# sachaMorin/dino

Hardware: AMD Instinct MI355X
Metric: frames/sec (480x480, ViT-S/8) DINOSeg inference (higher is better)
Workload: dtype fp16 (linears, Q.K^T; P.V bf16; fp32 accumulate)

## Files before the change

dino_amd/capi.py:

```python
from __future__ import annotations

import ctypes as C
import os
import re
from typing import Optional

import torch

_HERE = os.path.dirname(os.path.abspath(__file__))
LIB_PATH = os.path.join(_HERE, "lib", "libdinoseg_hip.so")
HEADER_PATH = os.path.join(os.path.dirname(_HERE), "include", "dinoseg.h")

BF16, BF16X3, FP16, FP16X3 = 0, 1, 2, 3
HEAD_LINEAR, HEAD_MLP = 0, 1
INPUT_U8_HWC, INPUT_F32_CHW = 0, 1
EPI_PLAIN, EPI_RESID, EPI_GELU, EPI_RELU = 0, 1, 2, 3
PROF_CLASSES = ("patch_embed", "layernorm", "qkv_gemm", "attention", "proj_gemm", "fc1_gemm", "fc2_gemm", "head", "attention_bwd")


class DinosegError(RuntimeError):
    pass


class Config(C.Structure):
# ... 54 lines not shown
                                              _i32, _i32, _i32, _f32, _i32, _i32, _vp]),
    "dinoseg_op_proj_pack_elems": (_i64, [_i32]),
    "dinoseg_op_pack_proj": (C.c_int, [_fp, _i32, _vp, _vp]),
    "dinoseg_op_proj_mlp_fused": (C.c_int, [_fp, _vp, _vp, _fp, _fp, _fp, _f32, _vp, _fp, _fp, _i32, _i32, _i32, _vp]),
    "dinoseg_op_pack_rs": (C.c_int, [_fp, _i32, _i32, _i32, _vp, _vp]),
    "dinoseg_op_gemm_rs": (C.c_int, [_vp, _i32, _vp, _fp, _i32, _i32, _i32, _i32, _fp, _vp, _i32, _vp, _vp, _vp, _i32, _i32, _i32, _f32, _vp]),
    "dinoseg_op_pack_rs_ln": (C.c_int, [_fp, _fp, _fp, _fp, _i32, _i32, _vp, _fp, _vp]),
    "dinoseg_op_ln_gemm_rs": (C.c_int, [_fp, _f32, _vp, _fp, _i32, _i32, _i32, _i32, _vp, _i32, _vp, _vp, _vp, _i32, _i32, _i32, _f32, _vp]),
    "dinoseg_op_mlp3_pack_elems": (_i64, [_i32, _i32]),
    "dinoseg_op_pack_mlp3": (C.c_int, [_fp, _fp, _fp, _fp, _fp, _fp, _fp, _fp, _fp, _fp, _i32, _i32, _i32, _vp, _vp]),
    "dinoseg_op_proj_mlp_fused3": (C.c_int, [_fp, _vp, _i64, _fp, _f32, _vp, _fp, _i32, _i32, _i32, _i32, _vp]),
    "dinoseg_op_mlp4_pack_elems": (_i64, [_i32, _i32]),
    "dinoseg_op_pack_mlp4": (C.c_int, [_fp, _fp, _fp, _fp, _fp, _fp, _fp, _fp, _fp, _fp, _i32, _i32, _i32, _vp, _vp]),
    "dinoseg_op_proj_mlp_fused4": (C.c_int, [_fp, _vp, _fp, _f32, _vp, _fp, _i32, _i32, _i32, _i32, _vp]),
    "dinoseg_op_block_tail_fused4": (C.c_int, [_fp, _vp, _fp, _f32, _vp, _fp, _vp, _vp, _vp, _i32, _i32, _i32, _i32, _f32, _i32, _i32, _i32, _vp]),
    "dinoseg_op_block_tail_fused3": (C.c_int, [_fp, _vp, _i64, _fp, _f32, _vp, _fp, _vp, _vp, _vp, _i64, _i32, _i32, _i32, _i32, _f32, _i32, _i32,
                                               _i32, _i32, _vp]),
    "dinoseg_op_attention": (C.c_int, [_vp, _vp, _vp, _i64, _vp, _i64, _fp, _i32, _i32, _i32, _i32, _i32, _vp]),
    "dinoseg_op_layernorm": (C.c_int, [_fp, _fp, _fp, _f32, _i32, _i32, _vp, _i64, _i32, _fp, _i32, _i32, _vp]),
    "dinoseg_op_pos_resample": (C.c_int, [_fp, _i32, _i32, _i32, _fp, _vp]),
    "dinoseg_op_patch_gather": (C.c_int, [_vp, _i32, _i32, _i32, _vp, _i64, _i32, _vp]),
    "dinoseg_op_head_final": (C.c_int, [_vp, _i64, _i32, _i32, _i32, _fp, _fp, _i32, _fp, _fp, _vp]),
    "dinoseg_op_head_wide": (C.c_int, [_vp, _i64, _i32, _i32, _i32, _vp, _i64, _fp, _i32, _fp, _fp, _vp]),
    "dinoseg_prepare_resolution_hw": (C.c_int, [_vp, _i32, _i32, _vp]),
    "dinoseg_forward_hw": (C.c_int, [_vp, _vp, _i32, _i32, _i32, _i32, _fp, _fp, _i32, _fp, _vp]),
    "dinoseg_last_selfattention_hw": (C.c_int, [_vp, _vp, _i32, _i32, _i32, _i32, _fp, _vp]),
    "dinoseg_forward_mask_hw": (C.c_int, [_vp, _vp, _i32, _i32, _i32, _fp, _i32, _fp, _fp, _vp]),
    "dinoseg_features_hw": (C.c_int, [_vp, _vp, _i32, _i32, _i32, _i32, _i32, _fp, _vp]),
    "dinoseg_train_forward_hw": (C.c_int, [_vp, _vp, _i32, _i32, _i32, _i32, _fp, _vp]),
    "dinoseg_train_step_hw": (C.c_int, [_vp, _vp, _i32, _i32, _i32, _i32, _fp, _fp, _fp, _vp]),
    "dinoseg_workspace_bytes_hw": (_i64, [_vp, _i32, _i32, _i32]),
    "dinoseg_op_pos_resample_hw": (C.c_int, [_fp, _i32, _i32, _i32, _i32, _fp, _vp]),
    "dinoseg_op_patch_gather_hw": (C.c_int, [_vp, _i32, _i32, _i32, _i32, _vp, _i64, _i32, _vp]),
}

_lib: Optional[C.CDLL] = None


def header_symbols() -> list:
    with open(HEADER_PATH) as f:
        text = re.sub(r"/\*.*?\*/", "", f.read(), flags=re.S)
    return sorted(set(re.findall(r"\b(dinoseg_[a-z0-9_]+)\s*\(", text)))


def lib() -> C.CDLL:
    global _lib
# ... 35 lines not shown
```

dino_amd/csrc/api.hip:

```cpp
#include <stdarg.h>
#include <stdio.h>
#include <string.h>

#include <map>
#include <string>
#include <vector>

#include "handle.h"

using namespace dseg;

static thread_local char g_err[1024] = "";

extern "C" void dinoseg_set_error(const char* fmt, ...) {
    va_list ap;
    va_start(ap, fmt);
    vsnprintf(g_err, sizeof(g_err), fmt, ap);
    va_end(ap);
}
extern "C" const char* dinoseg_last_error(void) { return g_err; }
extern "C" int dinoseg_version(void) { return 300; }

int device_cu_count() {
    static std::atomic<int> cache[64];
// ... 140 lines not shown
            return -1;
        }
        if (h->device != attr.device) {
            if (h->device >= 0) {
                DeviceGuard old(h);
                if (h->wbuf) (void)hipFree(h->wbuf);
                if (h->pos_cache) (void)hipFree(h->pos_cache);
                release_workspaces(h);
                (void)dinoseg_train_release(h);
                for (auto& e : h->stage_ev) (void)hipEventDestroy(e);
                h->stage_ev.clear();
                h->stage_done = 0;
                for (auto& r : h->prof_recs) {
                    (void)hipEventDestroy(r.a);
                    (void)hipEventDestroy(r.b);
                }
                h->prof_recs.clear();
                for (auto& e : h->prof_pool) (void)hipEventDestroy(e);
                h->prof_pool.clear();
                h->wbuf = nullptr; h->pos_cache = nullptr; h->pos_hp = h->pos_wp = -1;
                h->wbuf_bytes = h->pos_cap = 0;
                h->tws_B = h->tws_H = h->tws_W = h->tr_B = -1;
                h->packed.clear();
                h->packed_slab.clear();
                h->packed_mlp.clear();
                h->packed_proj.clear();
                h->packed_qkvf.clear();
                h->packed_mlp3.clear();
    h->packed_mlp4.clear();
    h->packed_rs_bias.clear();
                h->packed_mlp4.clear();
                h->packed_rs_bias.clear();
                h->packed_rs.clear();
                h->bound.clear();
                h->grads.clear();
            }
            h->device = attr.device;
        }
    }
    BoundTensor t;
    t.ptr = reinterpret_cast<const float*>(dev_ptr);
    t.shape.assign(shape, shape + ndim);
    h->bound[name] = t;
    h->weights_ready = false;
    h->pos_stale = true;
    return 0;
// ... 57 lines not shown
        if (ln_fed(sp)) total += align_up((size_t)gemm_ln_slab_elems(sp.N, sp.K, sp.planes) * sizeof(bf16_t), 256);
    }
    const int Dm = h->cfg.embed_dim, Fh = h->cfg.embed_dim * h->cfg.mlp_ratio;
    const bool mlp_fusable = mlp_fused_supported(Dm, Fh, h->planes);
    const bool mlp3_fusable = mlp_fused3_supported(Dm, Fh, h->planes);
    const bool mlp4_fusable = options().mlp_fused4 && mlp_fused4_supported(Dm, Fh, h->planes);
    auto rs_kind = [&](const LinSpec& sp) -> int {
        if (!options().gemm_rs || h->planes != 1 || Dm != 768 || sp.wname.rfind("dino.blocks.", 0) != 0) return -1;
        const int bit = sp.wname.find("mlp.fc1.weight") != std::string::npos ? 1 : sp.wname.find("attn.qkv.weight") != std::string::npos ? 2 : 4;
        if (!(options().gemm_rs & bit)) return -1;
        if (sp.K == 768 && (sp.wname.find("attn.qkv.weight") != std::string::npos || sp.wname.find("mlp.fc1.weight") != std::string::npos)) return 0;
        if (sp.N == 768 && sp.K % 192 == 0 && (sp.wname.find("attn.proj.weight") != std::string::npos || sp.wname.find("mlp.fc2.weight") != std::string::npos)) return 1;
        return -1;
    };
    auto rs_ln = [&](const LinSpec& sp) -> bool { return rs_kind(sp) == 0 && options().gemm_rs_ln; };
    for (const LinSpec& sp : specs)
        if (rs_kind(sp) >= 0) total += align_up((size_t)sp.N * sp.K * sizeof(bf16_t), 256) + (rs_ln(sp) ? align_up((size_t)sp.N * sizeof(float), 256) : 0);
    if (mlp3_fusable) total += (size_t)h->cfg.n_blocks * align_up((size_t)mlp_fused3_pack_elems(Dm, Fh) * sizeof(bf16_t), 256);
    if (mlp4_fusable) total += (size_t)h->cfg.n_blocks * align_up((size_t)mlp_fused4_pack_elems(Dm, Fh) * sizeof(bf16_t), 256);
    if (mlp_fusable)
        total += (size_t)h->cfg.n_blocks * (align_up((size_t)mlp_fused_pack_elems(Dm, Fh) * sizeof(bf16_t), 256) +
                                            align_up((size_t)mlp_fused_proj_pack_elems(Dm) * sizeof(bf16_t), 256) +
                                            align_up((size_t)mlp_fused_qkv_pack_elems(Dm) * sizeof(bf16_t), 256));
    if (total > h->wbuf_bytes) {
        ++h->generation;
        if (h->wbuf) DSEG_CHECK_HIP(hipFree(h->wbuf));
        h->wbuf = nullptr;
        DSEG_CHECK_HIP(hipMalloc(reinterpret_cast<void**>(&h->wbuf), total));
        h->wbuf_bytes = total;
    }
    size_t off = 0;
    std::vector<PackJob> jobs;
    for (const LinSpec& sp : specs) {
        PackedLinear pk;
        pk.w = reinterpret_cast<bf16_t*>(h->wbuf + off);
        pk.plane = (long)sp.n_pad * sp.k_pad;
        pk.n_pad = sp.n_pad;
        pk.k_pad = sp.k_pad;
        off += align_up((size_t)sp.planes * sp.n_pad * sp.k_pad * sizeof(bf16_t), 256);
        jobs.push_back({W(h, sp.wname), pk.w, pk.plane, sp.N, sp.K, sp.n_pad, sp.k_pad, sp.planes, 0, sp.fmt});
        if (sp.n_pad != sp.N) {
            pk.bias_pad = reinterpret_cast<float*>(h->wbuf + off);
            off += align_up((size_t)sp.n_pad * sizeof(float), 256);
            DSEG_CHECK_HIP(hipMemsetAsync(pk.bias_pad, 0, (size_t)sp.n_pad * sizeof(float), s));
            DSEG_CHECK_HIP(hipMemcpyAsync(pk.bias_pad, W(h, sp.bname), (size_t)sp.N * sizeof(float),
                                          hipMemcpyDeviceToDevice, s));
        }
        h->packed[sp.wname] = pk;
        if (ln_fed(sp)) {
            bf16_t* slab = reinterpret_cast<bf16_t*>(h->wbuf + off);
            off += align_up((size_t)gemm_ln_slab_elems(sp.N, sp.K, sp.planes) * sizeof(bf16_t), 256);
            DSEG_TRY(launch_pack_slabs(W(h, sp.wname), sp.N, sp.K, sp.planes, slab, s, sp.fmt));
            h->packed_slab[sp.wname] = slab;
        }
    }
    DSEG_TRY(launch_multi_pack(jobs.data(), (int)jobs.size(), s));
    h->packed_mlp.clear();
    h->packed_proj.clear();
    h->packed_qkvf.clear();
    h->packed_mlp3.clear();
    h->packed_rs.clear();
    for (const LinSpec& sp : specs)
        if (rs_kind(sp) >= 0) {
            bf16_t* dst = reinterpret_cast<bf16_t*>(h->wbuf + off);
            off += align_up((size_t)sp.N * sp.K * sizeof(bf16_t), 256);
            if (rs_ln(sp)) {
                float* fb = reinterpret_cast<float*>(h->wbuf + off);
                off += align_up((size_t)sp.N * sizeof(float), 256);
                const std::string blk = sp.wname.substr(0, sp.wname.find(sp.wname.find("attn.qkv") != std::string::npos ? "attn.qkv" : "mlp.fc1"));
                const std::string nrm = blk + (sp.wname.find("attn.qkv") != std::string::npos ? "norm1" : "norm2");
                DSEG_TRY(launch_pack_rs_ln(W(h, sp.wname), W(h, nrm + ".weight"), W(h, nrm + ".bias"), W(h, sp.bname), sp.N, sp.K, dst, fb, s, sp.fmt));
                h->packed_rs_bias[sp.wname] = fb;
            } else {
                DSEG_TRY(launch_pack_rs(W(h, sp.wname), sp.N, sp.K, rs_kind(sp), dst, s, sp.fmt));
            }
            h->packed_rs[sp.wname] = dst;
        }
    if (mlp3_fusable)
        for (int i = 0; i < h->cfg.n_blocks; ++i) {
// ... 445 lines not shown
            DSEG_PROF(DINOSEG_PROF_FC1, DSEG_TRY(gemm_any(g, b + "mlp.fc1.weight")));
        }
        }
        {
            const PackedLinear& pk = h->packed.at(b + "mlp.fc2.weight");
            GemmParams g = {};
            g.A = HB; g.a_plane = L.hb_plane; g.lda = F;
            g.W = pk.w; g.w_plane = pk.plane;
            g.M = L.M; g.N = D; g.K = F; g.planes = P; g.fmt = FM; g.epi = EPI_RESID; g.dispatch_rows = disp_M;
            g.bias = W(h, b + "mlp.fc2.bias");
            g.out_f32 = X; g.ldo_f32 = D;
            DSEG_PROF(DINOSEG_PROF_FC2, DSEG_TRY(gemm_any(g, b + "mlp.fc2.weight")));
        }
        }
        if (tap_block == i + 1 && tap_out) DSEG_CHECK_HIP(hipMemcpyAsync(tap_out, X, xbytes, hipMemcpyDeviceToDevice, s));
        if (mreq && mreq->feat_out && mreq->feat_blocks == i + 1 && i + 1 < c.n_blocks)
            return launch_layernorm(X, W(h, "dino.norm.weight"), W(h, "dino.norm.bias"), c.ln_eps, L.M, D, nullptr, 0, 1, mreq->feat_out, 0,
                                    L.ntok, s);
    }
    if (mreq && mreq->feat_out)
        return launch_layernorm(X, W(h, "dino.norm.weight"), W(h, "dino.norm.bias"), c.ln_eps, L.M, D, nullptr, 0, 1, mreq->feat_out, 0,
                                L.ntok, s);

    DSEG_PROF(DINOSEG_PROF_LN, DSEG_TRY(launch_layernorm(X, W(h, "dino.norm.weight"), W(h, "dino.norm.bias"), c.ln_eps, L.M, D, FEAT, L.feat_plane,
                              HP, nullptr, 1, L.ntok, s, SF)));

    if (c.head_kind == DINOSEG_HEAD_MLP) {
        {
            const PackedLinear& pk = h->packed.at("clf.layer_1.weight");
            GemmParams g = {};
            g.A = FEAT; g.a_plane = L.feat_plane; g.lda = D;
            g.W = pk.w; g.w_plane = pk.plane;
            g.M = L.Mp; g.N = 256; g.K = D; g.planes = HP; g.fmt = SF; g.epi = EPI_RELU;
            g.bias = pk.bias_pad;
            g.out_bf16 = H1; g.out_plane = L.h1_plane; g.ldo = 256;
            DSEG_PROF(DINOSEG_PROF_HEAD, DSEG_TRY(launch_gemm(g, s)));
        }
        {
            const PackedLinear& pk = h->packed.at("clf.layer_2.weight");
            GemmParams g = {};
            g.A = H1; g.a_plane = L.h1_plane; g.lda = 256;
            g.W = pk.w; g.w_plane = pk.plane;
            g.M = L.Mp; g.N = 128; g.K = 256; g.planes = HP; g.fmt = SF; g.epi = EPI_RELU;
            g.bias = pk.bias_pad;
            g.out_bf16 = H2; g.out_plane = L.h2_plane; g.ldo = 128;
            DSEG_PROF(DINOSEG_PROF_HEAD, DSEG_TRY(launch_gemm(g, s)));
// ... 577 lines not shown
extern "C" int dinoseg_op_patch_gather_hw(const void* x, int32_t x_kind, int32_t B, int32_t H, int32_t W, void* out, int64_t out_plane,
                                          int32_t planes, void* stream) {
    if (!frame_ok(H, W)) {
        dinoseg_set_error("Resolution should be a multiple of 8.");
        return -1;
    }
    float mean255[3], inv255[3];
    norm_consts(mean255, inv255);
    return launch_patch_gather(x, x_kind, B, H, W, mean255, inv255, reinterpret_cast<bf16_t*>(out), out_plane, planes,
                               reinterpret_cast<hipStream_t>(stream), planes == 2 ? options().op_fmt : FMT_BF16);
}

extern "C" int dinoseg_op_patch_gather(const void* x, int32_t x_kind, int32_t B, int32_t r, void* out, int64_t out_plane,
                                       int32_t planes, void* stream) {
    return dinoseg_op_patch_gather_hw(x, x_kind, B, r, r, out, out_plane, planes, stream);
}

extern "C" int dinoseg_op_head_final(const void* in, int64_t in_plane, int32_t ld, int32_t M, int32_t K, const float* Wc,
                                     const float* b, int32_t C, float* logp, int32_t* argmax, void* stream) {
    return launch_head_final(reinterpret_cast<const bf16_t*>(in), in_plane, ld, M, K, Wc, b, C, logp, argmax,
                             reinterpret_cast<hipStream_t>(stream), options().op_fmt);
}

extern "C" int dinoseg_op_head_wide(const void* in, int64_t in_plane, int32_t ld, int32_t M, int32_t K, const void* Wp, int64_t w_plane,
                                    const float* b, int32_t C, float* logp, int32_t* argmax, void* stream) {
    return launch_head_wide(reinterpret_cast<const bf16_t*>(in), in_plane, ld, M, K, reinterpret_cast<const bf16_t*>(Wp), w_plane, b, C,
                            logp, argmax, reinterpret_cast<hipStream_t>(stream), options().op_fmt);
}
```

dino_amd/csrc/common.h:

```cpp
#pragma once
#include <hip/hip_runtime.h>
#include <stdint.h>

namespace dseg {

typedef __attribute__((ext_vector_type(8))) __bf16 bf16x8;
typedef __attribute__((ext_vector_type(4))) __bf16 bf16x4;
typedef __attribute__((ext_vector_type(2))) __bf16 bf16x2;
typedef __attribute__((ext_vector_type(2))) float f32x2;
typedef __attribute__((ext_vector_type(4))) float f32x4;
typedef __attribute__((ext_vector_type(16))) float f32x16;

typedef uint16_t bf16_t;

constexpr int WAVE = 64;

__device__ __forceinline__ uint32_t pack_bf16x2(float a, float b) {
    f32x2 v = {a, b};
    return __builtin_bit_cast(uint32_t, __builtin_convertvector(v, bf16x2));
}
__device__ __forceinline__ float bf16_lo_to_f32(uint32_t packed) { return __builtin_bit_cast(float, packed << 16); }
__device__ __forceinline__ float bf16_hi_to_f32(uint32_t packed) { return __builtin_bit_cast(float, packed & 0xFFFF0000u); }
__device__ __forceinline__ float bf16_to_f32(bf16_t v) { return __builtin_bit_cast(float, (uint32_t)v << 16); }

// ... 68 lines not shown

__device__ __forceinline__ f32x16 mfma32(bf16x8 a, bf16x8 b, f32x16 c) {
    return __builtin_amdgcn_mfma_f32_32x32x16_bf16(a, b, c, 0, 0, 0);
}

template <int FMT>
__device__ __forceinline__ f32x16 mfma32f(bf16x8 a, bf16x8 b, f32x16 c) {
    if constexpr (FMT == FMT_FP16) return __builtin_amdgcn_mfma_f32_32x32x16_f16(__builtin_bit_cast(f16x8, a), __builtin_bit_cast(f16x8, b), c, 0, 0, 0);
    else return __builtin_amdgcn_mfma_f32_32x32x16_bf16(a, b, c, 0, 0, 0);
}

__device__ __forceinline__ bf16x8 lds_frag(const char* p) {
    return __builtin_bit_cast(bf16x8, *reinterpret_cast<const uint4*>(p));
}

__device__ __forceinline__ int acc_row(int r, int h) { return (r & 3) + 8 * (r >> 2) + 4 * h; }

__device__ __forceinline__ float wave_sum(float v) {
#pragma unroll
    for (int o = 32; o > 0; o >>= 1) v += __shfl_xor(v, o);
    return v;
}

__device__ __forceinline__ float gelu_erf(float x) {
    const float z = fabsf(x) * 0.70710678118654752440f;
    const float t = __builtin_amdgcn_rcpf(fmaf(0.3275911f, z, 1.0f));
    float pl = fmaf(1.061405429f, t, -1.453152027f);
    pl = fmaf(pl, t, 1.421413741f);
    pl = fmaf(pl, t, -0.284496736f);
    pl = fmaf(pl, t, 0.254829592f);
    const float pe = pl * t * __builtin_amdgcn_exp2f(-z * z * 1.44269504088896340736f);
    return 0.5f * x * (x >= 0.f ? 2.0f - pe : pe);
}

__device__ __forceinline__ float gelu_fast(float x) {
    const float xc = __builtin_amdgcn_fmed3f(x, -8.0f, 8.0f);
    const float u = xc * xc;
    float q = fmaf(1.01537542e-3f, u, -1.06782573e-1f);
    q = fmaf(q, u, -2.30111381f);
    const float e = __builtin_amdgcn_exp2f(q * xc);
    return x * __builtin_amdgcn_rcpf(1.0f + e);
}

__device__ __forceinline__ float gelu_erf_grad(float x) {
    const float z = fabsf(x) * 0.70710678118654752440f;
    const float t = __builtin_amdgcn_rcpf(fmaf(0.3275911f, z, 1.0f));
// ... 42 lines not shown
```

dino_amd/csrc/elementwise.hip:

```cpp
#include "common.h"
#include "kernels.h"

namespace dseg {

__global__ void pack_planes_kernel(const float* __restrict__ src, int rows, int cols, bf16_t* __restrict__ dst,
                                   long plane, int rows_pad, int cols_pad, int planes, int fmt) {
    const long total = (long)rows_pad * cols_pad;
    for (long i = (long)blockIdx.x * blockDim.x + threadIdx.x; i < total; i += (long)gridDim.x * blockDim.x) {
        const int r = (int)(i / cols_pad), c = (int)(i - (long)r * cols_pad);
        const float v = (r < rows && c < cols) ? src[(long)r * cols + c] : 0.f;
        bf16_t hi, lo;
        split1(v, fmt, hi, lo);
        dst[i] = hi;
        if (planes == 2) dst[plane + i] = lo;
    }
}

int launch_pack_planes(const float* src, int rows, int cols, bf16_t* dst, long plane, int rows_pad, int cols_pad,
                       int planes, hipStream_t s, int fmt) {
    const long total = (long)rows_pad * cols_pad;
    int grid = (int)((total + 255) / 256);
    if (grid > 2048) grid = 2048;
    hipLaunchKernelGGL(pack_planes_kernel, dim3(grid), dim3(256), 0, s, src, rows, cols, dst, plane, rows_pad, cols_pad, planes, fmt);
    DSEG_CHECK_HIP(hipGetLastError());
// ... 82 lines not shown
__global__ __launch_bounds__(256) void layernorm_kernel(const float* __restrict__ x, const float* __restrict__ gamma,
                                                        const float* __restrict__ beta, float eps, int M,
                                                        bf16_t* __restrict__ out, long out_plane, int planes,
                                                        float* __restrict__ out_f32, int drop_cls, int ntok, int fmt) {
    constexpr int D = 128 * NV;
    const int lane = threadIdx.x & 63;
    const int wid = blockIdx.x * 4 + (threadIdx.x >> 6);
    const int nw = gridDim.x * 4;
    f32x2 g[NV], bta[NV];
#pragma unroll
    for (int i = 0; i < NV; ++i) {
        g[i] = *reinterpret_cast<const f32x2*>(gamma + i * 128 + lane * 2);
        bta[i] = *reinterpret_cast<const f32x2*>(beta + i * 128 + lane * 2);
    }
    for (int m = wid; m < M; m += nw) {
        long orow = m;
        if (drop_cls) {
            const int b = m / ntok, t = m - b * ntok;
            if (t == 0) continue;
            orow = (long)b * (ntok - 1) + t - 1;
        }
        const float* xr = x + (long)m * D;
        f32x2 v[NV];
        float s = 0.f;
#pragma unroll
        for (int i = 0; i < NV; ++i) {
            v[i] = *reinterpret_cast<const f32x2*>(xr + i * 128 + lane * 2);
            s += v[i][0] + v[i][1];
        }
        const float mean = wave_sum(s) * (1.0f / D);
        float q = 0.f;
#pragma unroll
        for (int i = 0; i < NV; ++i) {
            v[i][0] -= mean;
            v[i][1] -= mean;
            q += v[i][0] * v[i][0] + v[i][1] * v[i][1];
        }
        const float rstd = 1.0f / sqrtf(wave_sum(q) * (1.0f / D) + eps);
#pragma unroll
        for (int i = 0; i < NV; ++i) {
            const float y0 = v[i][0] * rstd * g[i][0] + bta[i][0];
            const float y1 = v[i][1] * rstd * g[i][1] + bta[i][1];
            const long o = orow * D + i * 128 + lane * 2;
            if (out_f32) {
                f32x2 y = {y0, y1};
                *reinterpret_cast<f32x2*>(out_f32 + o) = y;
            }
            if (out) {
                uint32_t hi, lo;
                if (fmt == FMT_FP16) split2<FMT_FP16>(y0, y1, hi, lo);
                else split_bf16x2(y0, y1, hi, lo);
                *reinterpret_cast<uint32_t*>(out + o) = hi;
                if (planes == 2) *reinterpret_cast<uint32_t*>(out + out_plane + o) = lo;
            }
        }
    }
}

int launch_layernorm(const float* x, const float* gamma, const float* beta, float eps, int M, int D, bf16_t* out,
                     long out_plane, int planes, float* out_f32, int drop_cls, int ntok, hipStream_t s, int fmt) {
    if (M <= 0) return 0;
    if (D % 128 != 0 || D > 1024) {
        dinoseg_set_error("layernorm: D=%d must be a multiple of 128 and <= 1024", D);
        return -1;
    }
// ... 519 lines not shown
```

dino_amd/csrc/handle.h:

```cpp
#pragma once
#include <map>
#include <string>
#include <vector>

#include "../../include/dinoseg.h"
#include "common.h"
#include "kernels.h"

using namespace dseg;

#define DSEG_TRY(expr)            \
    do {                          \
        int _rc = (expr);         \
        if (_rc != 0) return _rc; \
    } while (0)

struct BoundTensor {
    const float* ptr = nullptr;
    std::vector<int64_t> shape;
};

struct PackedLinear {
    bf16_t* w = nullptr;
    long plane = 0;
    int n_pad = 0, k_pad = 0;
    float* bias_pad = nullptr;
};

struct dinoseg_handle {
    dinoseg_config cfg;
    int planes;
    int fmt = 0;
    int device = -1;
    std::map<std::string, BoundTensor> bound;
    std::map<std::string, std::vector<int64_t>> expected;
    char* wbuf = nullptr;
    size_t wbuf_bytes = 0;
    std::map<std::string, PackedLinear> packed;
    std::map<std::string, bf16_t*> packed_slab;
    std::map<std::string, bf16_t*> packed_mlp;
    std::map<std::string, bf16_t*> packed_proj;
    std::map<std::string, bf16_t*> packed_rs;
    std::map<std::string, float*> packed_rs_bias;
    std::map<std::string, bf16_t*> packed_mlp4;
    std::map<std::string, bf16_t*> packed_mlp3;
    std::map<std::string, bf16_t*> packed_qkvf;
    bool packed_mlp_stale = false;
    bool weights_ready = false;
    int fp16_patch_planes_snap = 1;
    int64_t generation = 0;
    float* pos_cache = nullptr;
    int pos_hp = -1, pos_wp = -1;
    bool pos_stale = false;
    size_t pos_cap = 0;
    char* ws = nullptr;
    size_t ws_bytes = 0;
    int ws_B = -1, ws_H = -1, ws_W = -1;
    char* ws2 = nullptr;
    size_t ws2_bytes = 0;
    int ws2_B = -1, ws2_H = -1, ws2_W = -1;
    hipStream_t aux_stream = nullptr;
    hipEvent_t ev_fork = nullptr, ev_join = nullptr;
    bool in_split = false;
    std::map<std::string, float*> grads;
    char* tws = nullptr;
    size_t tws_bytes = 0;
    int tws_B = -1, tws_H = -1, tws_W = -1;
    int tr_B = -1, tr_H = -1, tr_W = -1;
    int* bad_label_flag = nullptr;
// ... 83 lines not shown
```

dino_amd/csrc/kernels.h:

```cpp
#pragma once
#include <hip/hip_runtime.h>
#include <stdint.h>

namespace dseg {

typedef uint16_t bf16_t;

enum GemmEpilogue {
    EPI_PLAIN = 0,
    EPI_RESID = 1,
    EPI_GELU = 2,
    EPI_RELU = 3,
    EPI_QKV = 4,
    EPI_PATCH = 5,
    EPI_BF16 = 6,
    EPI_ATOMIC = 7,
    EPI_DGELU = 8,
    EPI_DRELU = 9,
};

struct GemmParams {
    const bf16_t* A; long a_plane; int lda;
    const bf16_t* W; long w_plane;
    int M, N, K;
// ... 147 lines not shown
int launch_attention_z(const AttnParams& p, hipStream_t s);
int launch_attention_za(const AttnParams& p, hipStream_t s);
bool attention_x3_za(int batch, int heads, int ntok);

int launch_pack_planes(const float* src, int rows, int cols, bf16_t* dst, long plane, int rows_pad, int cols_pad,
                       int planes, hipStream_t s, int fmt = 0);

int launch_layernorm(const float* x, const float* gamma, const float* beta, float eps, int M, int D,
                     bf16_t* out, long out_plane, int planes, float* out_f32, int drop_cls, int ntok, hipStream_t s, int fmt = 0);

int launch_patch_gather(const void* x, int kind, int B, int H, int W, const float* mean255, const float* inv_std255,
                        bf16_t* out, long out_plane, int planes, hipStream_t s, int fmt = 0);

int launch_cls_rows(float* X, const float* cls, const float* pos, int B, int ntok, int D, hipStream_t s);

int launch_pos_resample(const float* pos_embed, int g, int D, int oh, int ow, float* out, hipStream_t s);

constexpr int HEAD_FINAL_MAX_C = 32, HEAD_WIDE_MAX_C = 256;
int launch_head_final(const bf16_t* in, long in_plane, int ld, int M, int K, const float* W, const float* b, int C,
                      float* logp, int32_t* argmax, hipStream_t s, int fmt = 0, const bf16_t* Wp = nullptr, long w_plane = 0);
int launch_head_wide(const bf16_t* in, long in_plane, int ld, int M, int K, const bf16_t* Wp, long w_plane, const float* b, int C,
                     float* logp, int32_t* argmax, hipStream_t s, int fmt);

int launch_attn_probs(const bf16_t* q, const bf16_t* k, long plane, int planes, int B, int heads, int ntok, int npad, float* out,
                      hipStream_t s, int fmt = 0);
int launch_cls_mask_attn(const bf16_t* q, const bf16_t* k, const bf16_t* v, long plane, int planes, int heads, int ntok, int npad,
                         const float* mask, int n_masks, bf16_t* ctx, long ctx_plane, float* probs, hipStream_t s, int fmt = 0);
int launch_broadcast_row0(float* X, int D, int n, hipStream_t s);
int launch_resize_u8(const uint8_t* src, int sh, int sw, uint8_t* dst, int dh, int dw, hipStream_t s);
int launch_confusion(const int32_t* pred, const int64_t* gt, long n, int C, int64_t* cm, hipStream_t s);

struct AttnBwdParams {
    const bf16_t* q; const bf16_t* k; const bf16_t* v; long qkv_plane;
    const bf16_t* dO; const bf16_t* O; long dO_plane;
    const float* lse;
    float* neg_lse; float* neg_delta;
    bf16_t* dqkv; long dqkv_plane;
    int B, heads, ntok, npad, planes;
};
int launch_attention_bwd(const AttnBwdParams& p, hipStream_t s);

int launch_transpose_planes(const float* src_f32, const bf16_t* src_pl, long src_plane, int ld_src, int M, int C,
                            bf16_t* T, long t_plane, int c_pad, int m_pad, bf16_t* Nout, long n_plane, int ldn,
                            float* colsum, int planes, int drop_cls, int ntok, hipStream_t s, int det_region = 0);
int launch_nll_loss_grad(const float* logp, const int64_t* labels, const float* dlogp, int M, int C, float* acc, int* flags,
                         float* loss, bf16_t* dz, long dz_plane, int ldz, hipStream_t s);
// ... 36 lines not shown
```

include/dinoseg.h:

```cpp
#ifndef DINOSEG_H
#define DINOSEG_H

#include <stdint.h>

#ifdef __cplusplus
extern "C" {
#endif

typedef struct dinoseg_handle dinoseg_handle;

enum { DINOSEG_BF16 = 0, DINOSEG_BF16X3 = 1, DINOSEG_FP16 = 2, DINOSEG_FP16X3 = 3 };
enum { DINOSEG_HEAD_LINEAR = 0, DINOSEG_HEAD_MLP = 1 };
enum { DINOSEG_INPUT_U8_HWC = 0,
       DINOSEG_INPUT_F32_CHW = 1 };

typedef struct dinoseg_config {
    int32_t embed_dim;
    int32_t num_heads;
    int32_t n_blocks;
    int32_t patch;
    int32_t mlp_ratio;
    int32_t n_classes;
    int32_t head_kind;
    int32_t pos_grid;
// ... 145 lines not shown
                                const float* bqkv, const float* gamma1, const float* beta1, void* q, void* k, void* v, int32_t B,
                                int32_t ntok, int32_t npad, int32_t heads, float qscale, int32_t D, int32_t F, void* stream);

int dinoseg_op_attention(const void* q, const void* k, const void* v, int64_t qkv_plane, void* ctx, int64_t ctx_plane,
                         float* lse, int32_t B, int32_t heads, int32_t ntok, int32_t npad, int32_t planes, void* stream);

int dinoseg_op_layernorm(const float* x, const float* gamma, const float* beta, float eps, int32_t M, int32_t D,
                         void* out_bf16, int64_t out_plane, int32_t planes, float* out_f32, int32_t drop_cls,
                         int32_t ntok, void* stream);

int dinoseg_op_pos_resample(const float* pos_embed, int32_t g, int32_t D, int32_t o, float* out, void* stream);
int dinoseg_op_pos_resample_hw(const float* pos_embed, int32_t g, int32_t D, int32_t oh, int32_t ow, float* out, void* stream);

int dinoseg_op_patch_gather(const void* x, int32_t x_kind, int32_t B, int32_t r, void* out, int64_t out_plane,
                            int32_t planes, void* stream);
int dinoseg_op_patch_gather_hw(const void* x, int32_t x_kind, int32_t B, int32_t H, int32_t W, void* out, int64_t out_plane,
                               int32_t planes, void* stream);

int dinoseg_op_head_final(const void* in, int64_t in_plane, int32_t ld, int32_t M, int32_t K, const float* W,
                          const float* b, int32_t C, float* logp, int32_t* argmax, void* stream);
int dinoseg_op_head_wide(const void* in, int64_t in_plane, int32_t ld, int32_t M, int32_t K, const void* Wp, int64_t w_plane,
                         const float* b, int32_t C, float* logp, int32_t* argmax, void* stream);

int dinoseg_op_attention_bwd(const void* q, const void* k, const void* v, int64_t qkv_plane, const void* dO, const void* O,
                             int64_t o_plane, const float* lse, float* scratch, void* dqkv, int64_t dqkv_plane, int32_t B,
                             int32_t heads, int32_t ntok, int32_t npad, int32_t planes, void* stream);

int dinoseg_op_layernorm_bwd(const float* dy, const float* x, const float* gamma, float eps, int32_t M, int32_t D, float* dx,
                             int32_t accumulate, float* dgamma, float* dbeta, int32_t drop_cls, int32_t ntok, void* stream);

#ifdef __cplusplus
}
#endif
#endif
```

Before: 2569.

## Fuse final layernorm and MLP segmentation head into one persistent kernel

```diff
diff --git a/dino_amd/capi.py b/dino_amd/capi.py
--- a/dino_amd/capi.py
+++ b/dino_amd/capi.py
@@ -100,6 +100,9 @@
     "dinoseg_op_patch_gather": (C.c_int, [_vp, _i32, _i32, _i32, _vp, _i64, _i32, _vp]),
     "dinoseg_op_head_final": (C.c_int, [_vp, _i64, _i32, _i32, _i32, _fp, _fp, _i32, _fp, _fp, _vp]),
     "dinoseg_op_head_wide": (C.c_int, [_vp, _i64, _i32, _i32, _i32, _vp, _i64, _fp, _i32, _fp, _fp, _vp]),
+    "dinoseg_op_head_fused_pack_elems": (_i64, [_i32]),
+    "dinoseg_op_pack_head_fused": (C.c_int, [_vp, _i64, _vp, _i64, _i32, _vp, _vp]),
+    "dinoseg_op_head_fused": (C.c_int, [_fp, _fp, _fp, _f32, _i32, _i32, _i32, _vp, _fp, _fp, _fp, _fp, _i32, _fp, _fp, _vp]),
     "dinoseg_prepare_resolution_hw": (C.c_int, [_vp, _i32, _i32, _vp]),
     "dinoseg_forward_hw": (C.c_int, [_vp, _vp, _i32, _i32, _i32, _i32, _fp, _fp, _i32, _fp, _vp]),
     "dinoseg_last_selfattention_hw": (C.c_int, [_vp, _vp, _i32, _i32, _i32, _i32, _fp, _vp]),
diff --git a/dino_amd/csrc/api.hip b/dino_amd/csrc/api.hip
--- a/dino_amd/csrc/api.hip
+++ b/dino_amd/csrc/api.hip
@@ -186,6 +186,7 @@
                 h->wbuf_bytes = h->pos_cap = 0;
                 h->tws_B = h->tws_H = h->tws_W = h->tr_B = -1;
                 h->packed.clear();
+                h->packed_head = nullptr;
                 h->packed_slab.clear();
                 h->packed_mlp.clear();
                 h->packed_proj.clear();
@@ -289,6 +290,8 @@
         total += (size_t)h->cfg.n_blocks * (align_up((size_t)mlp_fused_pack_elems(Dm, Fh) * sizeof(bf16_t), 256) +
                                             align_up((size_t)mlp_fused_proj_pack_elems(Dm) * sizeof(bf16_t), 256) +
                                             align_up((size_t)mlp_fused_qkv_pack_elems(Dm) * sizeof(bf16_t), 256));
+    const bool head_fusable = h->cfg.head_kind == DINOSEG_HEAD_MLP && head_fused_supported(Dm, h->cfg.n_classes);
+    if (head_fusable) total += align_up((size_t)head_fused_pack_elems(Dm) * sizeof(bf16_t), 256);
     if (total > h->wbuf_bytes) {
         ++h->generation;
         if (h->wbuf) DSEG_CHECK_HIP(hipFree(h->wbuf));
@@ -322,6 +325,14 @@
         }
     }
     DSEG_TRY(launch_multi_pack(jobs.data(), (int)jobs.size(), s));
+    h->packed_head = nullptr;
+    if (head_fusable) {
+        h->packed_head = reinterpret_cast<bf16_t*>(h->wbuf + off);
+        off += align_up((size_t)head_fused_pack_elems(Dm) * sizeof(bf16_t), 256);
+        const PackedLinear& l1 = h->packed.at("clf.layer_1.weight");
+        const PackedLinear& l2 = h->packed.at("clf.layer_2.weight");
+        DSEG_TRY(launch_pack_head_fused(l1.w, l1.plane, l2.w, l2.plane, Dm, h->packed_head, s));
+    }
     h->packed_mlp.clear();
     h->packed_proj.clear();
     h->packed_qkvf.clear();
@@ -813,6 +824,18 @@
         return launch_layernorm(X, W(h, "dino.norm.weight"), W(h, "dino.norm.bias"), c.ln_eps, L.M, D, nullptr, 0, 1, mreq->feat_out, 0,
                                 L.ntok, s);
 
+    if (h->packed_head) {
+        HeadFusedParams g = {};
+        g.X = X; g.gamma = W(h, "dino.norm.weight"); g.beta = W(h, "dino.norm.bias"); g.eps = c.ln_eps;
+        g.ntok = L.ntok; g.Mp = L.Mp; g.D = D;
+        g.Wf = h->packed_head;
+        g.b1 = h->packed.at("clf.layer_1.weight").bias_pad; g.b2 = h->packed.at("clf.layer_2.weight").bias_pad;
+        g.W3 = W(h, "clf.layer_3.weight"); g.b3 = W(h, "clf.layer_3.bias"); g.C = c.n_classes;
+        g.logp = logp_out ? logp_out : reinterpret_cast<float*>(ws + L.HB); g.amax = argmax_out;
+        DSEG_PROF(DINOSEG_PROF_HEAD, DSEG_TRY(launch_head_fused(g, s, SF)));
+        return 0;
+    }
+
     DSEG_PROF(DINOSEG_PROF_LN, DSEG_TRY(launch_layernorm(X, W(h, "dino.norm.weight"), W(h, "dino.norm.bias"), c.ln_eps, L.M, D, FEAT, L.feat_plane,
                               HP, nullptr, 1, L.ntok, s, SF)));
 
@@ -1436,6 +1459,33 @@
                              reinterpret_cast<hipStream_t>(stream), options().op_fmt);
 }
 
+extern "C" int64_t dinoseg_op_head_fused_pack_elems(int32_t D) { return head_fused_supported(D, 1) ? head_fused_pack_elems(D) : -1; }
+
+extern "C" int dinoseg_op_pack_head_fused(const void* W1p, int64_t w1_plane, const void* W2p, int64_t w2_plane, int32_t D, void* dst,
+                                          void* stream) {
+    if (!W1p || !W2p || !dst) {
+        dinoseg_set_error("dinoseg_op_pack_head_fused: null pointer");
+        return -1;
+    }
+    return launch_pack_head_fused(reinterpret_cast<const bf16_t*>(W1p), w1_plane, reinterpret_cast<const bf16_t*>(W2p), w2_plane, D,
+                                  reinterpret_cast<bf16_t*>(dst), reinterpret_cast<hipStream_t>(stream));
+}
+
+extern "C" int dinoseg_op_head_fused(const float* x, const float* gamma, const float* beta, float eps, int32_t B, int32_t ntok, int32_t D,
+                                     const void* Wf, const float* b1, const float* b2, const float* W3, const float* b3, int32_t C,
+                                     float* logp, int32_t* argmax, void* stream) {
+    if (!x || !gamma || !beta || !Wf || !b1 || !b2 || !W3 || !b3 || !logp || B <= 0 || ntok < 2) {
+        dinoseg_set_error("dinoseg_op_head_fused: bad argument");
+        return -1;
+    }
+    HeadFusedParams g = {};
+    g.X = x; g.gamma = gamma; g.beta = beta; g.eps = eps;
+    g.ntok = ntok; g.Mp = B * (ntok - 1); g.D = D;
+    g.Wf = reinterpret_cast<const bf16_t*>(Wf); g.b1 = b1; g.b2 = b2; g.W3 = W3; g.b3 = b3; g.C = C;
+    g.logp = logp; g.amax = argmax;
+    return launch_head_fused(g, reinterpret_cast<hipStream_t>(stream), options().op_fmt);
+}
+
 extern "C" int dinoseg_op_head_wide(const void* in, int64_t in_plane, int32_t ld, int32_t M, int32_t K, const void* Wp, int64_t w_plane,
                                     const float* b, int32_t C, float* logp, int32_t* argmax, void* stream) {
     return launch_head_wide(reinterpret_cast<const bf16_t*>(in), in_plane, ld, M, K, reinterpret_cast<const bf16_t*>(Wp), w_plane, b, C,
diff --git a/dino_amd/csrc/common.h b/dino_amd/csrc/common.h
--- a/dino_amd/csrc/common.h
+++ b/dino_amd/csrc/common.h
@@ -114,6 +114,27 @@
     return v;
 }
 
+template <int NV>
+__device__ __forceinline__ void ln_row(f32x2 (&v)[NV], const f32x2 (&g)[NV], const f32x2 (&bta)[NV], float eps) {
+    constexpr int D = 128 * NV;
+    float s = 0.f;
+#pragma unroll
+    for (int i = 0; i < NV; ++i) s += v[i][0] + v[i][1];
+    const float mean = wave_sum(s) * (1.0f / D);
+    float q = 0.f;
+#pragma unroll
+    for (int i = 0; i < NV; ++i) {
+        v[i][0] -= mean;
+        v[i][1] -= mean;
+        q += v[i][0] * v[i][0] + v[i][1] * v[i][1];
+    }
+    const float rstd = 1.0f / sqrtf(wave_sum(q) * (1.0f / D) + eps);
+#pragma unroll
+    for (int i = 0; i < NV; ++i) {
+        v[i][0] = v[i][0] * rstd * g[i][0] + bta[i][0];
+        v[i][1] = v[i][1] * rstd * g[i][1] + bta[i][1];
+    }
+}
 __device__ __forceinline__ float gelu_erf(float x) {
     const float z = fabsf(x) * 0.70710678118654752440f;
     const float t = __builtin_amdgcn_rcpf(fmaf(0.3275911f, z, 1.0f));
diff --git a/dino_amd/csrc/elementwise.hip b/dino_amd/csrc/elementwise.hip
--- a/dino_amd/csrc/elementwise.hip
+++ b/dino_amd/csrc/elementwise.hip
@@ -128,25 +128,12 @@
         }
         const float* xr = x + (long)m * D;
         f32x2 v[NV];
-        float s = 0.f;
+#pragma unroll
+        for (int i = 0; i < NV; ++i) v[i] = *reinterpret_cast<const f32x2*>(xr + i * 128 + lane * 2);
+        ln_row<NV>(v, g, bta, eps);
 #pragma unroll
         for (int i = 0; i < NV; ++i) {
-            v[i] = *reinterpret_cast<const f32x2*>(xr + i * 128 + lane * 2);
-            s += v[i][0] + v[i][1];
-        }
-        const float mean = wave_sum(s) * (1.0f / D);
-        float q = 0.f;
-#pragma unroll
-        for (int i = 0; i < NV; ++i) {
-            v[i][0] -= mean;
-            v[i][1] -= mean;
-            q += v[i][0] * v[i][0] + v[i][1] * v[i][1];
-        }
-        const float rstd = 1.0f / sqrtf(wave_sum(q) * (1.0f / D) + eps);
-#pragma unroll
-        for (int i = 0; i < NV; ++i) {
-            const float y0 = v[i][0] * rstd * g[i][0] + bta[i][0];
-            const float y1 = v[i][1] * rstd * g[i][1] + bta[i][1];
+            const float y0 = v[i][0], y1 = v[i][1];
             const long o = orow * D + i * 128 + lane * 2;
             if (out_f32) {
                 f32x2 y = {y0, y1};
diff --git a/dino_amd/csrc/handle.h b/dino_amd/csrc/handle.h
--- a/dino_amd/csrc/handle.h
+++ b/dino_amd/csrc/handle.h
@@ -45,6 +45,7 @@
     std::map<std::string, bf16_t*> packed_mlp4;
     std::map<std::string, bf16_t*> packed_mlp3;
     std::map<std::string, bf16_t*> packed_qkvf;
+    bf16_t* packed_head = nullptr;
     bool packed_mlp_stale = false;
     bool weights_ready = false;
     int fp16_patch_planes_snap = 1;
diff --git a/dino_amd/csrc/head_fused.hip b/dino_amd/csrc/head_fused.hip
--- /dev/null
+++ b/dino_amd/csrc/head_fused.hip
@@ -0,0 +1,283 @@
+#include "common.h"
+#include "kernels.h"
+
+namespace dseg {
+
+namespace {
+constexpr int HF_ROWS = 64, HF_N1 = 256, HF_N2 = 128, HF_K3 = 100, HF_LD3 = 128;
+constexpr int HF_SH1 = HF_N1 * 2 + 16;
+constexpr int HF_SH2 = HF_LD3 + 4;
+constexpr int hf_sa(int D) { return D * 2 + 16; }
+constexpr int hf_area(int D) {
+    const int a = 2 * HF_ROWS * hf_sa(D), b = 2 * HF_ROWS * HF_SH1, c = HF_ROWS * HF_SH2 * 4;
+    return a > b ? (a > c ? a : c) : (b > c ? b : c);
+}
+}
+
+long head_fused_pack_elems(int D) { return 2L * HF_N1 * D + 2L * HF_N2 * HF_N1; }
+
+bool head_fused_supported(int D, int C) { return D % 128 == 0 && D >= 128 && D <= 384 && C >= 1 && C <= HEAD_FINAL_MAX_C; }
+
+__global__ void head_fused_pack_kernel(const bf16_t* __restrict__ w, long w_plane, int N, int K, bf16_t* __restrict__ out) {
+    const long total = 2L * N * K / 8;
+    for (long i = (long)blockIdx.x * blockDim.x + threadIdx.x; i < total; i += (long)gridDim.x * blockDim.x) {
+        const int lane = (int)(i & 63);
+        const long f = i >> 6;
+        const int KB = K / 16, NT = N / 32;
+        const int kb = (int)(f % KB), j = (int)((f / KB) % NT), pl = (int)(f / ((long)KB * NT));
+        const bf16_t* src = w + pl * w_plane + (long)(j * 32 + (lane & 31)) * K + kb * 16 + (lane >> 5) * 8;
+        *reinterpret_cast<uint4*>(out + i * 8) = *reinterpret_cast<const uint4*>(src);
+    }
+}
+
+int launch_pack_head_fused(const bf16_t* w1, long w1_plane, const bf16_t* w2, long w2_plane, int D, bf16_t* dst, hipStream_t s) {
+    if (D % 128 != 0 || D > 384) {
+        dinoseg_set_error("head_fused pack: D=%d must be a multiple of 128 and <= 384", D);
+        return -1;
+    }
+    const long n1 = 2L * HF_N1 * D / 8, n2 = 2L * HF_N2 * HF_N1 / 8;
+    hipLaunchKernelGGL(head_fused_pack_kernel, dim3((int)((n1 + 255) / 256)), dim3(256), 0, s, w1, w1_plane, HF_N1, D, dst);
+    hipLaunchKernelGGL(head_fused_pack_kernel, dim3((int)((n2 + 255) / 256)), dim3(256), 0, s, w2, w2_plane, HF_N2, HF_N1,
+                       dst + 2L * HF_N1 * D);
+    DSEG_CHECK_HIP(hipGetLastError());
+    return 0;
+}
+
+template <int FMT, int CMAX, int NV>
+__global__ __launch_bounds__(512, 1) void head_fused_kernel(HeadFusedParams p) {
+    constexpr int D = 128 * NV, KB1 = D / 16, KB2 = HF_N1 / 16, SA = hf_sa(D);
+    extern __shared__ __attribute__((aligned(16))) char smem[];
+    float* Ws = reinterpret_cast<float*>(smem + hf_area(D));
+    const int tid = threadIdx.x, lane = tid & 63;
+    const int wave = __builtin_amdgcn_readfirstlane(tid >> 6);
+    const int lr = lane & 31, lh = lane >> 5;
+    const int wr = wave & 1, wc = wave >> 1;
+    const int C = p.C, Mp = p.Mp, n = p.ntok - 1;
+    for (int i = tid; i < C * HF_LD3; i += 512) {
+        const int c = i / HF_LD3, k = i - c * HF_LD3;
+        Ws[i] = k < HF_K3 ? p.W3[c * HF_K3 + k] : 0.f;
+    }
+    f32x2 g[NV], bta[NV];
+#pragma unroll
+    for (int i = 0; i < NV; ++i) {
+        g[i] = *reinterpret_cast<const f32x2*>(p.gamma + i * 128 + lane * 2);
+        bta[i] = *reinterpret_cast<const f32x2*>(p.beta + i * 128 + lane * 2);
+    }
+    const uint4* W1 = reinterpret_cast<const uint4*>(p.Wf);
+    const uint4* W2 = W1 + 2L * HF_N1 * D / 8;
+    constexpr long W1_PLANE = (long)(HF_N1 / 32) * KB1 * 64, W2_PLANE = (long)(HF_N2 / 32) * KB2 * 64;
+    const int items = (Mp + HF_ROWS - 1) / HF_ROWS;
+
+    for (int item = blockIdx.x; item < items; item += gridDim.x) {
+        const int m0 = item * HF_ROWS;
+        {
+            f32x2 v[8][NV];
+#pragma unroll
+            for (int r = 0; r < 8; ++r) {
+                int m = m0 + wave * 8 + r;
+                m = m < Mp ? m : Mp - 1;
+                const int b = m / n, t = m - b * n;
+                const float* xr = p.X + ((long)b * p.ntok + 1 + t) * D;
+#pragma unroll
+                for (int i = 0; i < NV; ++i) v[r][i] = *reinterpret_cast<const f32x2*>(xr + i * 128 + lane * 2);
+            }
+#pragma unroll
+            for (int r = 0; r < 8; ++r) {
+                ln_row<NV>(v[r], g, bta, p.eps);
+                char* dst = smem + (wave * 8 + r) * SA;
+#pragma unroll
+                for (int i = 0; i < NV; ++i) {
+                    uint32_t hi, lo;
+                    split2<FMT>(v[r][i][0], v[r][i][1], hi, lo);
+                    *reinterpret_cast<uint32_t*>(dst + (i * 128 + lane * 2) * 2) = hi;
+                    *reinterpret_cast<uint32_t*>(dst + HF_ROWS * SA + (i * 128 + lane * 2) * 2) = lo;
+                }
+            }
+        }
+        __syncthreads();
+
+        f32x16 acc[2];
+#pragma unroll
+        for (int j = 0; j < 2; ++j)
+#pragma unroll
+            for (int r = 0; r < 16; ++r) acc[j][r] = 0.f;
+        {
+            uint4 bq[4][2][2];
+            auto ldb = [&](int kb, uint4 (&b)[2][2]) __attribute__((always_inline)) {
+#pragma unroll
+                for (int pl = 0; pl < 2; ++pl)
+#pragma unroll
+                    for (int j = 0; j < 2; ++j) b[pl][j] = W1[pl * W1_PLANE + ((long)(wc * 2 + j) * KB1 + kb) * 64 + lane];
+            };
+            const char* ar = smem + (wr * 32 + lr) * SA + lh * 16;
+            ldb(0, bq[0]);
+            ldb(1, bq[1]);
+            ldb(2, bq[2]);
+#pragma unroll 1
+            for (int kb0 = 0; kb0 < KB1; kb0 += 4) {
+#pragma unroll
+                for (int u = 0; u < 4; ++u) {
+                    const int kb = kb0 + u;
+                    if (kb + 3 < KB1) ldb(kb + 3, bq[(u + 3) & 3]);
+                    const bf16x8 ah = lds_frag(ar + kb * 32), al = lds_frag(ar + HF_ROWS * SA + kb * 32);
+#pragma unroll
+                    for (int j = 0; j < 2; ++j) {
+                        acc[j] = mfma32f<FMT>(al, __builtin_bit_cast(bf16x8, bq[u][0][j]), acc[j]);
+                        acc[j] = mfma32f<FMT>(ah, __builtin_bit_cast(bf16x8, bq[u][1][j]), acc[j]);
+                        acc[j] = mfma32f<FMT>(ah, __builtin_bit_cast(bf16x8, bq[u][0][j]), acc[j]);
+                    }
+                }
+            }
+        }
+        __syncthreads();
+#pragma unroll
+        for (int j = 0; j < 2; ++j) {
+            const int col = wc * 64 + j * 32 + lr;
+            const float bias = p.b1[col];
+#pragma unroll
+            for (int r = 0; r < 16; r += 2) {
+                uint32_t hi, lo;
+                split2<FMT, true>(fmaxf(acc[j][r] + bias, 0.f), fmaxf(acc[j][r + 1] + bias, 0.f), hi, lo);
+                char* d0 = smem + (wr * 32 + acc_row(r, lh)) * HF_SH1 + col * 2;
+                char* d1 = smem + (wr * 32 + acc_row(r + 1, lh)) * HF_SH1 + col * 2;
+                *reinterpret_cast<uint16_t*>(d0) = (uint16_t)(hi & 0xFFFFu);
+                *reinterpret_cast<uint16_t*>(d1) = (uint16_t)(hi >> 16);
+                *reinterpret_cast<uint16_t*>(d0 + HF_ROWS * HF_SH1) = (uint16_t)(lo & 0xFFFFu);
+                *reinterpret_cast<uint16_t*>(d1 + HF_ROWS * HF_SH1) = (uint16_t)(lo >> 16);
+            }
+        }
+        __syncthreads();
+
+        f32x16 acc2;
+#pragma unroll
+        for (int r = 0; r < 16; ++r) acc2[r] = 0.f;
+        {
+            uint4 bq[4][2];
+            auto ldb = [&](int kb, uint4 (&b)[2]) __attribute__((always_inline)) {
+#pragma unroll
+                for (int pl = 0; pl < 2; ++pl) b[pl] = W2[pl * W2_PLANE + ((long)wc * KB2 + kb) * 64 + lane];
+            };
+            const char* ar = smem + (wr * 32 + lr) * HF_SH1 + lh * 16;
+            ldb(0, bq[0]);
+            ldb(1, bq[1]);
+            ldb(2, bq[2]);
+#pragma unroll 1
+            for (int kb0 = 0; kb0 < KB2; kb0 += 4) {
+#pragma unroll
+                for (int u = 0; u < 4; ++u) {
+                    const int kb = kb0 + u;
+                    if (kb + 3 < KB2) ldb(kb + 3, bq[(u + 3) & 3]);
+                    const bf16x8 ah = lds_frag(ar + kb * 32), al = lds_frag(ar + HF_ROWS * HF_SH1 + kb * 32);
+                    acc2 = mfma32f<FMT>(al, __builtin_bit_cast(bf16x8, bq[u][0]), acc2);
+                    acc2 = mfma32f<FMT>(ah, __builtin_bit_cast(bf16x8, bq[u][1]), acc2);
+                    acc2 = mfma32f<FMT>(ah, __builtin_bit_cast(bf16x8, bq[u][0]), acc2);
+                }
+            }
+        }
+        __syncthreads();
+        float* H2 = reinterpret_cast<float*>(smem);
+        {
+            const int col = wc * 32 + lr;
+            const float bias = p.b2[col];
+#pragma unroll
+            for (int r = 0; r < 16; r += 2) {
+                uint32_t hi, lo;
+                split2<FMT, true>(fmaxf(acc2[r] + bias, 0.f), fmaxf(acc2[r + 1] + bias, 0.f), hi, lo);
+                H2[(wr * 32 + acc_row(r, lh)) * HF_SH2 + col] = lo_to_f32<FMT>(hi) + lo_to_f32<FMT>(lo);
+                H2[(wr * 32 + acc_row(r + 1, lh)) * HF_SH2 + col] = hi_to_f32<FMT>(hi) + hi_to_f32<FMT>(lo);
+            }
+        }
+        __syncthreads();
+
+        const int sub = tid & 15, grp = tid >> 4;
+#pragma unroll 1
+        for (int half = 0; half < 2; ++half) {
+            const int row = half * 32 + grp;
+            const long m = (long)m0 + row;
+            if (m >= Mp) break;
+            float xv[8];
+            {
+                const f32x4 x0 = *reinterpret_cast<const f32x4*>(H2 + row * HF_SH2 + sub * 8);
+                const f32x4 x1 = *reinterpret_cast<const f32x4*>(H2 + row * HF_SH2 + sub * 8 + 4);
+#pragma unroll
+                for (int e = 0; e < 4; ++e) {
+                    xv[e] = x0[e];
+                    xv[4 + e] = x1[e];
+                }
+            }
+            float z[CMAX];
+#pragma unroll
+            for (int c = 0; c < CMAX; ++c) {
+                if (c < C) {
+                    const float4 w0 = *reinterpret_cast<const float4*>(Ws + c * HF_LD3 + sub * 8);
+                    const float4 w1 = *reinterpret_cast<const float4*>(Ws + c * HF_LD3 + sub * 8 + 4);
+                    float a = 0.f;
+                    a = fmaf(xv[0], w0.x, a); a = fmaf(xv[1], w0.y, a); a = fmaf(xv[2], w0.z, a); a = fmaf(xv[3], w0.w, a);
+                    a = fmaf(xv[4], w1.x, a); a = fmaf(xv[5], w1.y, a); a = fmaf(xv[6], w1.z, a); a = fmaf(xv[7], w1.w, a);
+                    a += __shfl_xor(a, 1, 16); a += __shfl_xor(a, 2, 16); a += __shfl_xor(a, 4, 16); a += __shfl_xor(a, 8, 16);
+                    z[c] = a + p.b3[c];
+                } else {
+                    z[c] = -INFINITY;
+                }
+            }
+            float mx = z[0];
+            int am = 0;
+#pragma unroll
+            for (int c = 1; c < CMAX; ++c)
+                if (c < C && z[c] > mx) {
+                    mx = z[c];
+                    am = c;
+                }
+            float sum = 0.f;
+#pragma unroll
+            for (int c = 0; c < CMAX; ++c)
+                if (c < C) sum += expf(z[c] - mx);
+            const float lse = logf(sum);
+#pragma unroll
+            for (int c = 0; c < CMAX; ++c)
+                if (c < C && (c & 15) == sub) p.logp[m * C + c] = (z[c] - mx) - lse;
+            if (p.amax && sub == 0) p.amax[m] = am;
+        }
+        __syncthreads();
+    }
+}
+
+template <int FMT, int CMAX, int NV>
+static int launch_hf(const HeadFusedParams& p, hipStream_t s) {
+    constexpr int D = 128 * NV;
+    const size_t lds = (size_t)hf_area(D) + (size_t)CMAX * HF_LD3 * sizeof(float);
+    static PerDeviceOnce once;
+    if (once.first()) {
+        DSEG_CHECK_HIP(hipFuncSetAttribute(reinterpret_cast<const void*>(&head_fused_kernel<FMT, CMAX, NV>),
+                                           hipFuncAttributeMaxDynamicSharedMemorySize, (int)lds));
+        once.mark();
+    }
+    const int ncu = device_cu_count();
+    if (ncu <= 0) return -1;
+    const int items = (p.Mp + HF_ROWS - 1) / HF_ROWS;
+    const int grid = items < ncu ? items : ncu;
+    hipLaunchKernelGGL((head_fused_kernel<FMT, CMAX, NV>), dim3(grid), dim3(512), lds, s, p);
+    DSEG_CHECK_HIP(hipGetLastError());
+    return 0;
+}
+
+template <int FMT, int CMAX>
+static int launch_hf_d(const HeadFusedParams& p, hipStream_t s) {
+    switch (p.D) {
+        case 128: return launch_hf<FMT, CMAX, 1>(p, s);
+        case 256: return launch_hf<FMT, CMAX, 2>(p, s);
+        default: return launch_hf<FMT, CMAX, 3>(p, s);
+    }
+}
+
+int launch_head_fused(const HeadFusedParams& p, hipStream_t s, int fmt) {
+    if (p.Mp <= 0) return 0;
+    if (!head_fused_supported(p.D, p.C) || p.ntok < 2) {
+        dinoseg_set_error("head_fused: need D in {128, 256, 384} and 1 <= C <= %d (D=%d C=%d ntok=%d)", HEAD_FINAL_MAX_C, p.D, p.C, p.ntok);
+        return -1;
+    }
+    if (fmt == FMT_FP16) return p.C <= 8 ? launch_hf_d<FMT_FP16, 8>(p, s) : launch_hf_d<FMT_FP16, 32>(p, s);
+    return p.C <= 8 ? launch_hf_d<FMT_BF16, 8>(p, s) : launch_hf_d<FMT_BF16, 32>(p, s);
+}
+
+}
diff --git a/dino_amd/csrc/kernels.h b/dino_amd/csrc/kernels.h
--- a/dino_amd/csrc/kernels.h
+++ b/dino_amd/csrc/kernels.h
@@ -193,6 +193,26 @@
 int launch_head_wide(const bf16_t* in, long in_plane, int ld, int M, int K, const bf16_t* Wp, long w_plane, const float* b, int C,
                      float* logp, int32_t* argmax, hipStream_t s, int fmt);
 
+struct HeadFusedParams {
+    const float* X;
+    const float* gamma;
+    const float* beta;
+    float eps;
+    int ntok, Mp, D;
+    const bf16_t* Wf;
+    const float* b1;
+    const float* b2;
+    const float* W3;
+    const float* b3;
+    int C;
+    float* logp;
+    int32_t* amax;
+};
+bool head_fused_supported(int D, int C);
+long head_fused_pack_elems(int D);
+int launch_pack_head_fused(const bf16_t* w1, long w1_plane, const bf16_t* w2, long w2_plane, int D, bf16_t* dst, hipStream_t s);
+int launch_head_fused(const HeadFusedParams& p, hipStream_t s, int fmt);
+
 int launch_attn_probs(const bf16_t* q, const bf16_t* k, long plane, int planes, int B, int heads, int ntok, int npad, float* out,
                       hipStream_t s, int fmt = 0);
 int launch_cls_mask_attn(const bf16_t* q, const bf16_t* k, const bf16_t* v, long plane, int planes, int heads, int ntok, int npad,
diff --git a/include/dinoseg.h b/include/dinoseg.h
--- a/include/dinoseg.h
+++ b/include/dinoseg.h
@@ -191,6 +191,12 @@
 int dinoseg_op_head_wide(const void* in, int64_t in_plane, int32_t ld, int32_t M, int32_t K, const void* Wp, int64_t w_plane,
                          const float* b, int32_t C, float* logp, int32_t* argmax, void* stream);
 
+int64_t dinoseg_op_head_fused_pack_elems(int32_t D);
+int dinoseg_op_pack_head_fused(const void* W1p, int64_t w1_plane, const void* W2p, int64_t w2_plane, int32_t D, void* dst, void* stream);
+int dinoseg_op_head_fused(const float* x, const float* gamma, const float* beta, float eps, int32_t B, int32_t ntok, int32_t D,
+                          const void* Wf, const float* b1, const float* b2, const float* W3, const float* b3, int32_t C,
+                          float* logp, int32_t* argmax, void* stream);
+
 int dinoseg_op_attention_bwd(const void* q, const void* k, const void* v, int64_t qkv_plane, const void* dO, const void* O,
                              int64_t o_plane, const float* lse, float* scratch, void* dqkv, int64_t dqkv_plane, int32_t B,
                              int32_t heads, int32_t ntok, int32_t npad, int32_t planes, void* stream);
```

After: 2580 (median of 6 runs). About the same (+0.4%).
